# nanoporetech/vbz_compression

Hardware: AMD Instinct MI355X
Metric: MB/s encode+decode, int16 signal, 1/2/4/8 MI355X vs CPU; ratio preserved (higher is better)
Workload: dtype int16

## Files before the change

### vbz_compression_amd/csrc/vbz_api.hip

```cpp
#include <hip/hip_runtime.h>

#include <cmath>
#include <cstdarg>
#include <cstdio>
#include <cstdlib>
#include <cstring>
#include <condition_variable>
#include <mutex>
#include <string>
#include <map>
#include <vector>

#include "../../include/vbz.h"
#include "../../include/vbz_gpu.h"
#include "vbz_kernels.h"

using namespace vbzhip;


struct ProfEntry
{
    const char* name;
    uint32_t launches;
    double ms;
// ... 1905 lines not shown
VBZ_EXPORT int vbz_gpu_x_svb_handover(vbz_gpu_ctx* c, const vbz_gpu_batch* bt, void* plans_out)
{
    if (!c || !bt || !plans_out) return -1;
    DeviceGuard dg(c->device);
    const uint32_t n = bt->n_reads;
    if (n == 0) return 0;
    hipStream_t s = c->stream;
    ReadBatch rb = to_rb(bt);
    uint32_t num, den;
    svb_factor(2, true, &num, &den);
    const size_t scratch_need = (size_t)(((unsigned __int128)bt->src_bytes * num + den - 1) / den) + (size_t)n * 96 + 256;
    StageSlots m;
    if (!ensure(c, c->scratch, scratch_need) || !ensure(c, c->meta, m.carve(nullptr, n)) || !ensure(c, c->encplan, zstd_encode_plan_bytes(n))) return -1;
    m.carve(c->meta.p, n);
    uint64_t* const svb_off = m.svb_off;
    uint32_t *const svb_cap = m.svb_cap, *const svb_size = m.svb_size, *const gate = m.gate;
    HIPCHK(c, launch_plan_scratch(n, bt->src_size, num, den, c->scratch.cap, svb_off, svb_cap, gate, false, s), "plan launch");
    ReadBatch a = rb;
    a.dst = (uint8_t*)c->scratch.p;
    a.dst_off = svb_off;
    a.dst_cap = svb_cap;
    a.result = svb_size;
    a.gate = gate;
    HIPCHK(c, launch_svb_encode(a, 2, true, 0, false, false, nullptr, c->encplan.p, s), "svb_encode launch");
    ReadBatch cp = rb;
    cp.src = (const uint8_t*)c->scratch.p;
    cp.src_off = svb_off;
    cp.src_size = svb_size;
    cp.gate = gate;
    HIPCHK(c, launch_copy_bytes(cp, 0, s), "copy launch");
    HIPCHK(c, hipMemcpyAsync(plans_out, c->encplan.p, (size_t)n * sizeof(EncPlan), hipMemcpyDeviceToDevice, s), "plan copy");
    return 0;
}
#endif

void vbz_gpu_profile_enable(vbz_gpu_ctx* c, int enable)
{
    if (!c) return;
    if (!enable) drain_profile(c);
    c->profiling = enable != 0;
    if (c->half) vbz_gpu_profile_enable(c->half, enable);
}

int vbz_gpu_decode_span_paths(vbz_gpu_ctx* c, uint32_t* by_spans)
{
    if (!c) return -1;
    DeviceGuard guard(c->device);
    if (by_spans) *by_spans = 0;
    if (c->last_span_frames == 0) return 0;
    std::vector<uint32_t> redo(c->last_span_frames);
    if (hipMemcpyAsync(redo.data(), c->last_span_redo, 4ull * redo.size(), hipMemcpyDeviceToHost, c->stream) != hipSuccess) return -1;
    if (hipStreamSynchronize(c->stream) != hipSuccess) return -1;
    uint32_t nb = 0;
    for (uint32_t v : redo) nb += v == 0;
    if (by_spans) *by_spans = nb;
    return (int)c->last_span_frames;
}

static int decode_paths_one(vbz_gpu_ctx* c, uint32_t* batched, uint32_t* walked);

int vbz_gpu_decode_paths(vbz_gpu_ctx* c, uint32_t* batched, uint32_t* walked)
{
    if (!c) return -1;
    uint32_t b0 = 0, w0 = 0, b1 = 0, w1 = 0;
    const int n0 = decode_paths_one(c, &b0, &w0);
    const int n1 = (n0 >= 0 && c->last_split && c->half) ? decode_paths_one(c->half, &b1, &w1) : 0;
// ... 417 lines not shown
```

### vbz_compression_amd/csrc/vbz_kernels.h

```cpp
#pragma once

#include <hip/hip_runtime.h>
#include <stdint.h>

namespace vbzhip {

constexpr uint32_t E_ZSTD = 0xFFFFFFFFu;
constexpr uint32_t E_INPUT_SIZE = 0xFFFFFFFEu;
constexpr uint32_t E_INTEGER_SIZE = 0xFFFFFFFDu;
constexpr uint32_t E_DESTINATION_SIZE = 0xFFFFFFFCu;
constexpr uint32_t E_STREAM = 0xFFFFFFFBu;
constexpr uint32_t E_VERSION = 0xFFFFFFFAu;
constexpr uint32_t E_OOM = 0xFFFFFFF9u;
constexpr uint32_t E_DEVICE = 0xFFFFFFF8u;
constexpr uint32_t E_FIRST = E_DEVICE;
constexpr uint32_t GATE_SKIP = E_FIRST - 1u;
constexpr int PHASE_SLOTS = 12;

constexpr uint32_t SIG_NONE = 0, SIG_F32 = 1, SIG_F16 = 2, SIG_BF16 = 3;
constexpr uint32_t SIG_CHUNK = 4;
constexpr uint32_t SIG_COUNT = 8;
constexpr uint32_t SIG_RANGE = 16;
constexpr uint32_t SIG_TRIM = 32;
constexpr uint32_t RANGE_STATS_RANGE = 0, RANGE_STATS_READ = 1;
// ... 246 lines not shown
    const RefLits* lits = nullptr;
    const uint32_t* lits_pos = nullptr;
    uint32_t lits_units = 0;
};

size_t zstd_ref_pre_bytes(uint32_t n_reads);
const RefPre* zstd_ref_pre(const void* pre_meta);
size_t zstd_ref_table_bytes(uint32_t n_reads);
hipError_t launch_zstd_ref_chain(const ReadBatch& b, const uint32_t* redo, void* pre_meta, void* tables, void* recs, uint64_t recs_cap, RefChains* out,
                                 hipStream_t s);
hipError_t launch_zstd_decode_only(const ReadBatch& b, uint32_t toosmall_code, const void* seq_dtables, const uint32_t* only, RefChains chains,
                                   unsigned long long* dbg, hipStream_t s);
size_t zstd_fast_meta_bytes(uint32_t n_reads);
const RefLits* zstd_ref_lits(const void* lit_meta, uint32_t n_reads);
bool zstd_ref_literals_enabled();
const uint32_t* zstd_fast_redo(const void* meta, uint32_t n_reads);
struct RefWork
{
    void *pre = nullptr, *tables = nullptr, *recs = nullptr;
    uint64_t recs_cap = 0;
    void* lits = nullptr;
    uint32_t lit_units = 0;
};
struct FastDecodeArgs
{
    uint32_t toosmall_code = 0;
    const void* seq_dtables = nullptr;
    void* meta = nullptr;
    RefWork ref;
    unsigned long long* dbg = nullptr;
    FastSide side;
};
hipError_t launch_zstd_decode_fast(const ReadBatch& b, const FastDecodeArgs& a, hipStream_t s);
size_t zstd_ref_lit_meta_bytes(uint32_t n_reads);
uint32_t zstd_ref_lit_units();
const uint32_t* zstd_ref_lit_skip(const void* lit_meta, uint32_t n_reads);
size_t seq_dtables_bytes();
void seq_dtables_build(void* host_buffer);
struct SpanDecodeArgs
{
    uint32_t toosmall_code = 0;
    const void* seq_dtables = nullptr;
    uint64_t content_bytes = 0;
    void* meta = nullptr;
    const uint32_t* redo = nullptr;
};
size_t zstd_dspan_meta_bytes(uint64_t content_bytes, uint32_t n_reads);
hipError_t launch_zstd_decode_spans(const ReadBatch& b, SpanDecodeArgs* a, hipStream_t s);

hipError_t launch_xxh64_batch(const uint8_t* src, const uint64_t* off, const uint32_t* len, const uint32_t* gate, const uint32_t* skip, uint32_t n,
                              uint64_t* out, hipStream_t s);
hipError_t launch_xxh64_verify(const ReadBatch& b, hipStream_t s);
hipError_t launch_checksum_insert(const ReadBatch& b, const uint64_t* hash, uint32_t hdr, const uint32_t* raw_size, uint32_t integer_size, hipStream_t s);

hipError_t launch_pack_layout(uint32_t n, const uint32_t* result, const uint64_t* dst_off, const uint32_t* dst_cap, uint64_t dst_bytes, uint32_t align,
                              uint64_t* packed_off, uint32_t* packed_size, hipStream_t s);
hipError_t launch_sized_layout(uint32_t n, const uint8_t* src, const uint64_t* src_off, const uint32_t* src_size, uint64_t src_bytes, uint32_t align,
                               uint32_t* raw_size, uint64_t* raw_off, hipStream_t s);
hipError_t launch_pack_gather(uint32_t n, const uint8_t* dst, const uint64_t* dst_off, const uint64_t* packed_off, const uint32_t* packed_size,
                              uint8_t* packed, uint64_t packed_cap, hipStream_t s);

hipError_t launch_plan_scratch(uint32_t n, const uint32_t* raw_size, uint32_t mul_num, uint32_t mul_den, uint64_t limit,
                               uint64_t* off, uint32_t* cap, uint32_t* gate, bool gate_is_input, hipStream_t s);
struct ScratchPlan
{
    uint32_t num, den;
// ... 108 lines not shown
```

### vbz_compression_amd/csrc/zstd_decode_fast.hip

```cpp
#include <algorithm>
#include <cstdlib>

#include "vbz_kernels.h"
#include "zstd_runs.h"
#include "zstd_frame.h"
#include "zstd_tables.h"

namespace vbzhip {

namespace {

constexpr uint32_t FAST_TASKS = 64;
constexpr uint32_t TASK_REL = 1u << 31, TASK_TAB = 1u << 30, TASK_CNT = TASK_TAB - 1u;

struct FastFrame
{
    uint32_t fcs, ntask, ntree, block_max;
    uint32_t tree_off[2], tree_len[2];
    uint32_t tlog[2], nw[2];
    uint32_t seq_off, seq_len, nseq;
    uint32_t b0_regen, base_out;
    uint32_t ws_lit, ws_pairs;
    uint32_t cp_off, cp_count, cp_spacing;
    uint32_t blk, lit_csize;
// ... 813 lines not shown
                    if (k0 + 1024u * c + 16u <= mq) v[u][c] = *(gl4*)(f + k0 + 1024u * c);
                const uint32_t rb = mq & 15u;
                tailb[u] = (uint32_t)lane < rb ? f[mq - rb + (uint32_t)lane] : 0u;
            }
#pragma unroll
            for (int u = 0; u < MG; ++u) {
                const uint32_t mq = (uint32_t)__builtin_amdgcn_readlane((int)m, g + u);
                gu8* d = (gu8*)dst + (uint32_t)__builtin_amdgcn_readlane((int)dpos, g + u);
#pragma unroll
                for (int c = 0; c < 3; ++c)
                    if (k0 + 1024u * c + 16u <= mq) *(gst4*)(d + k0 + 1024u * c) = v[u][c];
                const uint32_t rb = mq & 15u;
                if ((uint32_t)lane < rb) d[mq - rb + (uint32_t)lane] = (uint8_t)tailb[u];
                if (mq > 3072u + 16u) {
                    gcu8* f = (gcu8*)(tb + (uint64_t)(g + u) * pcap);
                    for (uint32_t k = k0 + 3072u; k + 16u <= mq; k += 1024u) *(gst4*)(d + k) = *(gl4*)(f + k);
                }
            }
        }
        res.tail = tail_end;
    } else if (F->noseq) {
        LEAVE();
    }
    res.blk = F->blk;
    res.regen = regen;
    res.csize = F->lit_csize;
    res.at = F->ws_lit;
    res.tb = (uint32_t)(tb - (uint64_t)dst);
    res.pcap = pcap;
    LEAVE();
#undef LEAVE
}

constexpr uint32_t RUNS_LDS = 8704;
__global__ __launch_bounds__(WAVE) void fast_runs_kernel(ReadBatch b, const FastFrame* frames, const SeqDTables* dtabs, uint32_t* redo)
{
    __shared__ __attribute__((aligned(16))) uint32_t lds[RUNS_LDS / 4];
    const int lane = threadIdx.x;
    const uint32_t r = blockIdx.x;
    if (redo[r]) return;
    const FastFrame* F = frames + r;
    const uint32_t nseq = F->nseq;
    if (nseq == 0) return;
    const uint8_t* src = b.src + b.src_off[r];
    uint8_t* dst = b.dst + b.dst_off[r];
    const uint2 llt = dtabs->ll[lane], mlt = dtabs->ml[lane];
    uint2* pairs = reinterpret_cast<uint2*>(dst + F->ws_pairs);
    const uint32_t regen = F->b0_regen, base_out = F->base_out;
    uint32_t total = 0, ok = 3;
    if (F->cp_count)
        ok = zero_run_chain_segments(src + F->seq_off, F->seq_len, pairs, nseq, llt, mlt, regen, src + F->cp_off, F->cp_count, F->cp_spacing, lane, &total, lds,
                                     RUNS_LDS);
    if (ok == 3) ok = zero_run_chain(src + F->seq_off, F->seq_len, pairs, nseq, llt, mlt, 6, 6, regen, lane, &total);
    if (ok != 1 || total != base_out) {
        if (lane == 0) redo[r] = 1;
        return;
    }
    __syncthreads();
    const uint32_t end = place_zero_runs(dst, pairs, nseq, dst + F->ws_lit, 2u, regen, 0u, F->fcs, F->block_max, reinterpret_cast<uint8_t*>(lds), RUNS_LDS - 8u, lane);
    if (lane == 0) {
        if (end != base_out) redo[r] = 1;
        else b.result[r] = F->fcs;
    }
}

}

static uint32_t ref_units_max()
{
    static const uint32_t v = [] {
        const char* e = getenv("VBZ_HIP_REF_UNITS");
        const int k = e ? atoi(e) : (int)4;
        return (uint32_t)(k < 1 ? 1 : (k > 4 ? 4 : k));
    }();
    return v;
}

static int ref_lits_ahead()
{
    static const int on = [] {
        const char* e = getenv("VBZ_HIP_REF_LITERALS");
        return e ? atoi(e) : 1;
    }();
    return on;
}

size_t zstd_fast_meta_bytes(uint32_t n_reads)
{
    return (size_t)n_reads * (sizeof(FastFrame) + FAST_TASKS * sizeof(FastTask) + 512 + 4 + 4) + 1024;
}

struct FastMeta
{
    FastFrame* frames;
    FastTask* tasks;
    uint8_t* weights;
    uint32_t* redo;
    uint32_t* scanned;
};
// ... 132 lines not shown
```

### vbz_compression_amd/csrc/zstd_encode.hip

```cpp
#include "vbz_kernels.h"
#include "zstd_entropy.h"
#include "zstd_frame.h"

namespace vbzhip {

namespace {

constexpr int WAVE = 64;
constexpr uint32_t BLOCK_MAX = 128u << 10;
constexpr uint32_t MIN_BLOCK = 4096;
constexpr uint32_t HUF_BLOCK_MAX = 92u << 10;
constexpr uint32_t SPLIT_MIN = 2048;
constexpr int MAXBLK = 16;
#ifndef VBZ_SPAN_BLOCK_KB
#define VBZ_SPAN_BLOCK_KB 16
#endif
constexpr uint32_t SPAN_BLOCK = VBZ_SPAN_BLOCK_KB << 10;
#ifndef VBZ_SPAN_SMALL_BLOCKS
#define VBZ_SPAN_SMALL_BLOCKS 2
#endif
constexpr uint32_t SPAN_BYTES_SMALL = SPAN_BLOCK * VBZ_SPAN_SMALL_BLOCKS, SPAN_BYTES_LARGE = SPAN_BLOCK * MAXBLK;
constexpr uint32_t SPAN_LARGE_FROM = 256u << 20;
#ifndef VBZ_KEYSPAN_KB
#define VBZ_KEYSPAN_KB 8
// ... 1246 lines not shown
    }
}

__device__ __forceinline__ void span_table_role(EncLds& L, SpanRegion* R, int lane)
{
    const uint32_t ns = R->nshared;
    if (ns == 0) return;
    uint32_t mine = 0;
#pragma unroll
    for (int j = 0; j < 4; ++j) {
        const uint32_t c = R->hist[lane + 64 * j];
        L.hist[lane + 64 * j] = c;
        mine += c;
    }
    const uint32_t D = wave_sum_u32(mine);
    wave_lds_sync();
    const uint32_t per = (D + ns - 1) / ns;
    region_plan(L, D, D, ns * ((per + SPAN_BLOCK - 1) / SPAN_BLOCK), lane);
    wave_lds_sync();
#pragma unroll
    for (int j = 0; j < 4; ++j) {
        const uint2 e = L.ctable[lane + 64 * j];
        R->ctable[lane + 64 * j] = e.x | (e.y << 16);
    }
    if (lane < 34) R->tree[lane] = reinterpret_cast<const uint32_t*>(L.tree)[lane];
    if (lane == 0) {
        R->mode = L.mode;
        R->treeSize = (uint32_t)L.treeSize;
        R->huffLog = L.huffLog;
    }
}

#ifndef VBZ_ENC_PACK_WAVES
#define VBZ_ENC_PACK_WAVES 5
#endif
#ifndef VBZ_PACK_PREFETCH
#define VBZ_PACK_PREFETCH 1
#endif
#ifndef VBZ_ENC_WAVES
#define VBZ_ENC_WAVES 4
#endif

template <bool TIMED, bool DEEP, bool TABLES = false>
__global__ __launch_bounds__(WAVE, VBZ_ENC_WAVES) void zstd_encode_kernel(ReadBatch b, const uint32_t* orig_size, uint32_t key_elem,
                                                           const uint32_t* key_bytes, uint32_t hdr, unsigned long long* dbg,
                                                           const uint32_t* src_cap, const SeqCTables* seqtab, const EncSpan* spans,
                                                           const uint32_t* span_count, uint8_t* span_tmp, uint32_t* span_size,
                                                           uint32_t* span_trail, uint32_t trailers, uint32_t* deep_d, EncPlan* plans, uint32_t* redo,
                                                           SpanShared shared)
{
    __shared__ __attribute__((aligned(16))) EncLds L;
    if (TABLES && shared.regions && blockIdx.x >= shared.first_block) {
        span_table_role(L, shared.regions + (blockIdx.x - shared.first_block), threadIdx.x);
        return;
    }
    unsigned long long tph[PHASE_SLOTS] = {};
    unsigned long long tlast = TIMED ? __builtin_readcyclecounter() : 0;
#define PHASE(k) do { if (TIMED) { unsigned long long tn = __builtin_readcyclecounter(); tph[k] += tn - tlast; tlast = tn; } } while (0)
    const int lane = threadIdx.x;
    const bool span_mode = spans != nullptr;
    EncSpan sp = {};
    if (span_mode) {
        if (blockIdx.x >= *span_count) return;
        sp = spans[blockIdx.x];
        if (sp.flags & SPAN_SHARED) return;
        if (lane == 0) { span_size[blockIdx.x] = 0; span_trail[blockIdx.x] = 0; }
        if (sp.flags & SPAN_SKIP) return;
// ... 815 lines not shown
            if (!jsingle) {
                uint8_t* tp = bp + 3 + lh + tsz;
                put_le(tp, s0, 2);
                put_le(tp + 2, s1, 2);
                put_le(tp + 4, s2, 2);
            }
        }
    };
    uint32_t ocur = opos;
    uint32_t spos = 0;
    uint32_t curblk = 0xFFFFFFFFu;
    if (st < 4 * nb) load_chunk(s_beg(st), s_cnt(st), 0, cur);
    PPHASE(1);
    uint32_t base_bits = 0;
    uint32_t flushed = 0;
    uint32_t cb = 0;
    uint32_t pend_fq = 0;
    uint8_t* pend_dst = nullptr;
    auto flush_pending = [&]() {
        uint4* pq = reinterpret_cast<uint4*>(L.obuf[cb ^ 1u]);
        for (uint32_t q = lane; q < pend_fq; q += WAVE) {
            const uint4 v = pq[q];
            pq[q] = make_uint4(0u, 0u, 0u, 0u);
            __builtin_memcpy(pend_dst + 16u * q, &v, 16);
        }
        pend_fq = 0;
    };
    while (st < 4 * nb) {
        if ((st >> 2) != curblk) {
            curblk = st >> 2;
            const uint32_t tsz = curblk == 0 ? treeSize : 0u;
            const uint32_t hl = 3u + blk_lh(curblk) + tsz + (blk_bs(curblk) < 256u ? 0u : 6u);
            if ((uint64_t)ocur + hl > limit) REDO();
            for (uint32_t i = lane; i < tsz; i += WAVE) out[ocur + 3u + blk_lh(curblk) + i] = reinterpret_cast<const uint8_t*>(L.tree)[i];
            spos = ocur + hl;
        }
        const uint32_t scnt = s_cnt(st);
        uint8_t* sop = out + spos;
        uint32_t nst = st, ndone = done + STEP_SYMS;
        if (ndone >= scnt) {
            ndone = 0;
            ++nst;
            while (nst < 4 * nb && s_cnt(nst) == 0) ++nst;
        }
        flush_pending();
#if VBZ_PACK_PREFETCH
        if (nst < 4 * nb) load_chunk(s_beg(nst), s_cnt(nst), ndone, nxt);
#endif
        const int32_t room = (int32_t)(scnt - done) - STEP_LANE * lane;
        const int skip = room >= STEP_LANE ? 0 : (room <= 0 ? STEP_LANE : (int)(STEP_LANE - room));
        uint32_t ent[STEP_LANE];
#pragma unroll
        for (int k = 0; k < STEP_LANE; ++k) ent[k] = mytable[(cur[k >> 2] >> (8 * (k & 3))) & 0xFF];
        if (skip != 0) {
#pragma unroll
            for (int k = 0; k < STEP_LANE; ++k) ent[k] = k >= skip ? ent[k] : 0u;
        }
        uint32_t Tb = 0;
#pragma unroll
        for (int k = 0; k < STEP_LANE; ++k) Tb += ent[k];
        Tb >>= 16;
        const uint32_t incl = wave_incl_scan_u32(Tb);
        const uint32_t total = (uint32_t)__builtin_amdgcn_readlane((int)incl, 63);
        const uint32_t allbits = base_bits + total;
        const uint32_t fq = allbits >> 7;
        if ((uint64_t)spos + flushed + 16ull * fq + 24 > limit) REDO();
        PPHASE(2);
// ... 66 lines not shown
#pragma unroll
        for (int k = 0; k < STEP_DW; ++k) cur[k] = nxt[k];
#else
        if (nst < 4 * nb) load_chunk(s_beg(nst), s_cnt(nst), ndone, cur);
#endif
        st = nst;
        done = ndone;
        PPHASE(5);
    }
    flush_pending();
    if (seqmode && curblk != 0xFFFFFFFFu) {
        wave_lds_sync();
        if ((uint64_t)spos + seqBytes > seqOff) REDO();
        for (uint32_t i = 16u * (uint32_t)lane; i < seqBytes; i += 16u * WAVE) {
            uint4 v;
            __builtin_memcpy(&v, out + seqOff + i, 16);
            if (i + 16u <= seqBytes) __builtin_memcpy(out + spos + i, &v, 16);
            else {
                const uint32_t w[4] = { v.x, v.y, v.z, v.w };
                for (uint32_t k = i; k < seqBytes; ++k) out[spos + k] = (uint8_t)(w[(k - i) >> 2] >> (8 * ((k - i) & 3)));
            }
        }
        wave_lds_sync();
        block_headers(curblk, ocur, seqBytes);
        ocur = spos + seqBytes;
    }
    opos = ocur;
    return true;
#undef PPHASE
#undef REDO
}

template <bool TIMED>
__global__ __launch_bounds__(WAVE, VBZ_ENC_PACK_WAVES) void zstd_pack_kernel(ReadBatch b, const uint32_t* orig_size, uint32_t key_elem, const uint32_t* key_bytes,
                                                                             uint32_t hdr, uint32_t trailers, const EncPlan* plans, uint32_t* redo,
                                                                             unsigned long long* dbg_)
{
    unsigned long long* const dbg = TIMED ? dbg_ : nullptr;
    __shared__ __attribute__((aligned(16))) PackLds L;
    unsigned long long tph[PHASE_SLOTS] = {};
    unsigned long long tlast = TIMED ? __builtin_readcyclecounter() : 0;
#define PPHASE(k) do { if (TIMED) { unsigned long long tn = __builtin_readcyclecounter(); tph[k] += tn - tlast; tlast = tn; } } while (0)
    const int lane = threadIdx.x;
    const uint32_t r = blockIdx.x;
    if (redo[r] != PLAN_READY) return;
#define REDO()                          \
    do {                                \
        if (lane == 0) redo[r] = 0;     \
        return;                         \
    } while (0)
    const uint32_t N = b.src_size[r];
    const uint32_t cap = b.dst_cap[r];
    const uint8_t* in = b.src + b.src_off[r];
    uint8_t* out = b.dst + b.dst_off[r];
    const EncPlan* FP = &plans[r];
    uint32_t K = 0;
    if (N >= SPLIT_MIN) {
        if (key_bytes) K = key_bytes[r];
        else if (key_elem) K = (orig_size[r] / key_elem + 3u) >> 2;
        if (K >= N) K = 0;
    }
    const uint32_t seqBytes = FP->seqBytes, seqOff = FP->seqOff;
    const uint32_t limit = seqBytes ? seqOff : cap;
    uint32_t opos = 0;
    if ((uint64_t)hdr + 9 > limit) REDO();
    if (lane == 0) {
        if (hdr) put_le(out, orig_size[r], 4);
        uint8_t* p = out + hdr;
        put_le(p, ZSTD_MAGIC, 4);
        if (N < 256) { p[4] = 0x20; p[5] = (uint8_t)N; }
        else if (N < 65536 + 256) { p[4] = 0x60; put_le(p + 5, N - 256, 2); }
        else { p[4] = 0xA0; put_le(p + 5, N, 4); }
    }
    opos = hdr + 5 + (N < 256 ? 1 : (N < 65536 + 256 ? 2 : 4));
    PPHASE(0);
    for (int region = 0; region < 2; ++region) {
        if (region == 1 && K == 0) break;
        const uint32_t r0 = region == 0 ? 0u : K;
        const uint32_t r1 = region == 0 ? (K ? K : N) : N;
        const EncRegionPlan* P = &FP->reg[region];
        const uint32_t S = P->S, Sh = P->Sh;
        const uint32_t opos_region = opos;
        if (!pack_region<TIMED>(L, in + r0, r0, out, opos, limit, P->ctable, P->tree, S, P->nblk, P->treeSize, P->seqmode != 0, r1 == N, seqBytes, seqOff, lane,
                                tph, tlast))
            REDO();
        if (Sh != S && opos - opos_region > S + (S >> 6) + 256u) REDO();
        PPHASE(6);
    }
    if (FP->cpCount != 0 && (trailers & 1u)) {
        const uint32_t count = FP->cpCount, tb = 8u + 4u + 4u * count + 4u;
        if ((uint64_t)opos + tb <= cap) {
            __syncthreads();
            uint8_t* tp = out + opos;
            if (lane == 0) {
                put_le(tp, CP_MAGIC, 4);
                put_le(tp + 4, tb - 8u, 4);
                put_le(tp + 8, FP->cpSpacing | (count << 16), 4);
                put_le(tp + 12 + 4 * count, tb, 4);
            }
            if ((uint32_t)lane < count) put_le(tp + 12 + 4 * lane, FP->cp[lane], 4);
            opos += tb;
        }
    }
    if (lane == 0) b.result[r] = opos;
    PPHASE(7);
    if (TIMED && lane == 0)
        for (int k = 0; k < PHASE_SLOTS; ++k) dbg[(size_t)r * PHASE_SLOTS + k] = tph[k];
#undef PPHASE
#undef REDO
}


__global__ __launch_bounds__(1024) void zstd_span_plan_kernel(uint32_t n, const uint32_t* svb_size, const uint32_t* orig_size, uint32_t key_elem,
                                                              const uint32_t* gate, uint32_t seq_enabled, uint32_t max_spans, uint64_t tmp_limit,
                                                              EncSpan* spans, uint32_t* span_first, uint32_t* span_count, SpanRegion* regions, uint32_t shspan)
{
// ... 82 lines not shown
                EncSpan e = {};
                e.read = base + q;
                bool keyseq = false;
                if (j < kN) {
                    e.r0 = (uint32_t)((uint64_t)qK * j / kN);
                    e.r1 = (uint32_t)((uint64_t)qK * (j + 1) / kN);
                    keyseq = keyseq1;
                    e.tmp_off = q_off[q] + (uint64_t)j * slotK;
                    e.tmp_cap = slotK;
                } else {
                    const uint32_t t = j - kN;
                    e.r0 = qK + (uint32_t)((uint64_t)D * t / dN);
                    e.r1 = qK + (uint32_t)((uint64_t)D * (t + 1) / dN);
                    e.tmp_off = q_off[q] + (uint64_t)kN * slotK + (uint64_t)t * slotD;
                    e.tmp_cap = slotD;
                    keyseq = dataseq;
                    if (q_shared[q]) e.flags = SPAN_SHARED | (t == 0 ? SPAN_TREE : 0u);
                }
                e.flags |= (j == 0 ? SPAN_FIRST : 0u) | (j + 1 == cntq ? SPAN_LAST : 0u) | (keyseq ? SPAN_KEYSEQ : 0u);
                e.ord = j;
                spans[si + j] = e;
            }
        }
        __syncthreads();
        if (tid == 1023) { carry_c = pc + ci; carry_b = pb + bi; }
        __syncthreads();
    }
    if (tid == 0) {
        span_first[n] = carry_c;
        *span_count = carry_c < max_spans ? carry_c : max_spans;
    }
}

__global__ __launch_bounds__(WAVE, VBZ_ENC_PACK_WAVES) void zstd_span_pack_kernel(ReadBatch b, const EncSpan* spans, const uint32_t* span_count, uint8_t* span_tmp,
                                                                                  uint32_t* span_size, uint32_t* span_trail, const SpanRegion* regions)
{
    __shared__ __attribute__((aligned(16))) PackLds L;
    const int lane = threadIdx.x;
    if (blockIdx.x >= *span_count) return;
    const EncSpan sp = spans[blockIdx.x];
    if ((sp.flags & (SPAN_SHARED | SPAN_SKIP)) != SPAN_SHARED) return;
    const SpanRegion* R = &regions[sp.read];
    const uint8_t* in = b.src + b.src_off[sp.read];
    uint8_t* out = span_tmp + sp.tmp_off;
    const uint32_t S = sp.r1 - sp.r0, cap = sp.tmp_cap;
    const uint32_t nblk = (S + SPAN_BLOCK - 1) / SPAN_BLOCK;
    const bool last = (sp.flags & SPAN_LAST) != 0, tree = (sp.flags & SPAN_TREE) != 0;
    const uint32_t mode = R->mode;
    uint32_t opos = 0;
    bool packed = false;
    if (mode == 2u) {
        unsigned long long tph[PHASE_SLOTS] = {}, tlast = 0;
        packed = pack_region<false>(L, in + sp.r0, sp.r0, out, opos, cap, R->ctable, R->tree, S, nblk, tree ? R->treeSize : 0u, false, last, 0u, 0u, lane, tph, tlast);
        if (packed && !tree && opos > S + 3u * nblk) packed = false;
        if (!packed && tree) {
            if (lane == 0) { span_size[blockIdx.x] = E_ZSTD; span_trail[blockIdx.x] = 0; }
            return;
        }
    }
    if (!packed) {
        if ((uint64_t)S + 3ull * nblk > cap) {
            if (lane == 0) { span_size[blockIdx.x] = E_ZSTD; span_trail[blockIdx.x] = 0; }
            return;
        }
        wave_lds_sync();
        const uint32_t base = S / nblk, extra = S % nblk;
        const bool rle = mode == 1u;
// ... 366 lines not shown
```

### vbz_compression_amd/csrc/zstd_runs.h

```cpp
#pragma once
#include "vbz_kernels.h"

namespace vbzhip {
namespace {

constexpr int WAVE = 64;
constexpr uint32_t BLOCK_MAX = 128u << 10;

__device__ const int16_t LL_DEFAULT[36] = { 4, 3, 2, 2, 2, 2, 2, 2, 2, 2, 2, 2, 2, 1, 1, 1, 2, 2,
                                            2, 2, 2, 2, 2, 2, 2, 3, 2, 1, 1, 1, 1, 1, -1, -1, -1, -1 };
__device__ const int16_t ML_DEFAULT[53] = { 1, 4, 3, 2, 2, 2, 2, 2, 2, 1, 1, 1, 1, 1, 1, 1, 1, 1, 1, 1, 1, 1, 1, 1, 1, 1, 1,
                                            1, 1, 1, 1, 1, 1, 1, 1, 1, 1, 1, 1, 1, 1, 1, 1, 1, 1, 1, -1, -1, -1, -1, -1, -1, -1 };
__device__ const int16_t OF_DEFAULT[29] = { 1, 1, 1, 1, 1, 1, 2, 2, 2, 1, 1, 1, 1, 1, 1, 1, 1, 1, 1, 1, 1, 1, 1, 1, -1, -1, -1, -1, -1 };
__device__ const uint32_t LL_BASE[36] = { 0, 1, 2, 3, 4, 5, 6, 7, 8, 9, 10, 11, 12, 13, 14, 15, 16, 18,
                                          20, 22, 24, 28, 32, 40, 48, 64, 128, 256, 512, 1024, 2048, 4096, 8192, 16384, 32768, 65536 };
__device__ const uint8_t LL_BITS[36] = { 0, 0, 0, 0, 0, 0, 0, 0, 0, 0, 0, 0, 0, 0, 0, 0, 1, 1,
                                         1, 1, 2, 2, 3, 3, 4, 6, 7, 8, 9, 10, 11, 12, 13, 14, 15, 16 };
__device__ const uint32_t ML_BASE[53] = { 3, 4, 5, 6, 7, 8, 9, 10, 11, 12, 13, 14, 15, 16, 17, 18, 19, 20,
                                          21, 22, 23, 24, 25, 26, 27, 28, 29, 30, 31, 32, 33, 34, 35, 37, 39, 41,
                                          43, 47, 51, 59, 67, 83, 99, 131, 259, 515, 1027, 2051, 4099, 8195, 16387, 32771, 65539 };
__device__ const uint8_t ML_BITS[53] = { 0, 0, 0, 0, 0, 0, 0, 0, 0, 0, 0, 0, 0, 0, 0, 0, 0, 0, 0, 0, 0, 0, 0, 0, 0, 0, 0,
                                         0, 0, 0, 0, 0, 1, 1, 1, 1, 2, 2, 3, 3, 4, 4, 5, 7, 8, 9, 10, 11, 12, 13, 14, 15, 16 };

__device__ __forceinline__ int hbit(uint32_t v) { return 31 - __clz((int)v); }
__device__ __forceinline__ uint32_t uni(uint32_t v) { return (uint32_t)__builtin_amdgcn_readfirstlane((int)v); }
__device__ __forceinline__ uint32_t lane_get(uint32_t v, uint32_t l) { return (uint32_t)__builtin_amdgcn_readlane((int)v, (int)l); }

__device__ __noinline__ uint32_t place_zero_runs(uint8_t* dst, const uint2* pairs, uint32_t nseq, const uint8_t* litp, uint32_t ltype,
                                    uint32_t regen, uint32_t opos, uint32_t fcs, uint32_t block_max, uint8_t* lds_lit,
                                    uint32_t lds_cap, int lane)
{
    const uint8_t rle_byte = ltype == 1 ? litp[0] : 0;
    uint32_t lposw = 0, oposw = opos;
    uint2 pnext = (uint32_t)lane < nseq ? pairs[lane] : make_uint2(0u, 0u);
    for (uint32_t base = 0; base < nseq; base += WAVE) {
        const uint32_t ll = pnext.x, ml = pnext.y;
        {
            const uint32_t i1 = base + WAVE + (uint32_t)lane;
            pnext = i1 < nseq ? pairs[i1] : make_uint2(0u, 0u);
        }
        const uint32_t il = wave_incl_scan_u32(ll), it = wave_incl_scan_u32(ll + ml);
        const uint32_t tl = (uint32_t)__builtin_amdgcn_readlane((int)il, 63), tt = (uint32_t)__builtin_amdgcn_readlane((int)it, 63);
        if ((uint64_t)lposw + tl > regen || (uint64_t)oposw + tt > fcs) return 0xFFFFFFFFu;
        const uint32_t lit_room = (tl + 15u) & ~15u;
        if (ltype != 1 && 5u * lit_room + tt + 16u <= lds_cap) {
            uint32_t* lds_sh = reinterpret_cast<uint32_t*>(lds_lit + lit_room);
            uint8_t* lds_out = lds_lit + 5u * lit_room;
            wave_lds_sync();
            for (uint32_t j = lane; 4 * j < tl; j += WAVE) {
                uint32_t v;
                __builtin_memcpy(&v, litp + lposw + 4 * j, 4);
                reinterpret_cast<uint32_t*>(lds_lit)[j] = v;
            }
            for (uint32_t j = 4u * (uint32_t)lane; j < lit_room; j += 4u * WAVE) *reinterpret_cast<uint4*>(lds_sh + j) = make_uint4(0u, 0u, 0u, 0u);
            for (uint32_t j = 16u * (uint32_t)lane; j < tt; j += 16u * WAVE) *reinterpret_cast<uint4*>(lds_out + j) = make_uint4(0u, 0u, 0u, 0u);
            wave_lds_sync();
            const uint32_t lo = il - ll, oo = it - (ll + ml);
            const uint32_t mprev = wave_prev_lane_u32(ml);
            if (ll != 0 && lane != 0) lds_sh[lo] = mprev;
            wave_lds_sync();
            uint32_t carry = 0;
            for (uint32_t j0 = 0; j0 < tl; j0 += 8u * WAVE) {
                const uint32_t j = j0 + 8u * (uint32_t)lane;
                uint32_t sh[8], run = 0;
                const uint4 a0 = j < lit_room ? *reinterpret_cast<const uint4*>(lds_sh + j) : make_uint4(0u, 0u, 0u, 0u);
                const uint4 a1 = j + 4 < lit_room ? *reinterpret_cast<const uint4*>(lds_sh + j + 4) : make_uint4(0u, 0u, 0u, 0u);
                const uint32_t dl[8] = { a0.x, a0.y, a0.z, a0.w, a1.x, a1.y, a1.z, a1.w };
#pragma unroll
                for (int k = 0; k < 8; ++k) {
                    run += dl[k];
                    sh[k] = run;
                }
                const uint32_t inc = wave_incl_scan_u32(run);
                const uint32_t before = carry + inc - run;
                uint2 lb = make_uint2(0u, 0u);
                if (j < lit_room) lb = *reinterpret_cast<const uint2*>(lds_lit + j);
#pragma unroll
                for (int k = 0; k < 8; ++k)
                    if (j + k < tl) lds_out[j + k + before + sh[k]] = (uint8_t)((k < 4 ? lb.x : lb.y) >> (8 * (k & 3)));
                carry += (uint32_t)__builtin_amdgcn_readlane((int)inc, 63);
            }
            wave_lds_sync();
            if (ll != 0) {
                const uint8_t lastb = lds_lit[il - 1];
                if (lastb != 0)
                    for (uint32_t k = 0; k < ml; ++k) lds_out[oo + ll + k] = lastb;
            }
            wave_lds_sync();
            uint8_t* g = dst + oposw;
            for (uint32_t j = 16u * (uint32_t)lane; j < tt; j += 16u * WAVE) {
                if (j + 16u <= tt) {
                    const uint4 v = *reinterpret_cast<const uint4*>(lds_out + j);
                    __builtin_memcpy(g + j, &v, 16);
                } else {
                    for (uint32_t k = j; k < tt; ++k) g[k] = lds_out[k];
                }
            }
            lposw += tl;
            oposw += tt;
            continue;
// ... 20 lines not shown
                dst[my_out + k] = lastb;
            }
        }
        my_out += ll;
        if (ml < 64) {
            const uint32_t v4 = (uint32_t)lastb * 0x01010101u;
            uint32_t k = 0;
            for (; k + 4 <= ml; k += 4) __builtin_memcpy(dst + my_out + k, &v4, 4);
            for (; k < ml; ++k) dst[my_out + k] = lastb;
        }
        uint64_t big = __ballot(ml >= 64);
        while (big) {
            const int sl_ = __ffsll((long long)big) - 1;
            big &= big - 1;
            const uint32_t bo = (uint32_t)__builtin_amdgcn_readlane((int)my_out, sl_);
            const uint32_t bl = (uint32_t)__builtin_amdgcn_readlane((int)ml, sl_);
            const uint32_t bv = (uint32_t)__builtin_amdgcn_readlane((int)lastb, sl_);
            for (uint32_t k = lane; k < bl; k += WAVE) dst[bo + k] = (uint8_t)bv;
        }
        lposw += tl;
        oposw += tt;
    }
    const uint32_t rest = regen - lposw;
    if ((uint64_t)oposw + rest > fcs) return 0xFFFFFFFFu;
    if (ltype == 1) {
        for (uint32_t k = lane; k < rest; k += WAVE) dst[oposw + k] = rle_byte;
    } else {
        for (uint32_t k = lane; k < rest; k += WAVE) dst[oposw + k] = litp[lposw + k];
    }
    oposw += rest;
    if (oposw - opos > BLOCK_MAX || oposw - opos > block_max) return 0xFFFFFFFFu;
    return oposw;
}

struct SeqDTables
{
    uint2 ll[64], ml[64];
};


__device__ __noinline__ uint32_t zero_run_chain(const uint8_t* bs_, uint32_t bsn_, uint2* ws, uint32_t nseq_, uint2 llt, uint2 mlt,
                                                uint32_t log_ll_, uint32_t log_ml_, uint32_t regen_, int lane, uint32_t* total_out)
{
    const uint32_t bsn = uni(bsn_), nseq = uni(nseq_), log_ll = uni(log_ll_), log_ml = uni(log_ml_), regen = uni(regen_);
    const uint8_t* bs = reinterpret_cast<const uint8_t*>(((uint64_t)uni((uint32_t)((uint64_t)bs_ >> 32)) << 32) |
                                                         uni((uint32_t)(uint64_t)bs_));
    if (bsn == 0) return 0u;
    uint32_t k0 = 0;
    auto load_window = [&]() -> uint32_t {
        const int64_t off = (int64_t)bsn - 4 * (int64_t)(k0 + (uint32_t)lane + 1);
        uint32_t v = 0;
        if (off >= 0) {
            __builtin_memcpy(&v, bs + off, 4);
        } else if (off > -4) {
            for (int k = 0; k < 4 + (int)off; ++k) v |= (uint32_t)bs[k] << (8 * (k - (int)off));
        }
        return v;
    };
    uint32_t win = load_window();
    const uint32_t top = lane_get(win, 0) >> 24;
    if (top == 0) return 0u;
    const uint32_t hb = (uint32_t)hbit(top);
    int64_t bits_left = (int64_t)(bsn - 1) * 8 + hb;
    uint64_t buf = 0;
    uint32_t have = 0, q = 0;
    auto refill = [&]() {
        if (have <= 32) {
            if (q - k0 == 64) {
                k0 += 64;
                win = load_window();
            }
            const uint32_t d = lane_get(win, q - k0);
            ++q;
            buf |= (uint64_t)d << (32 - have);
            have += 32;
// ... 11 lines not shown
    have -= 8 - hb;
    refill();
    uint32_t sl = take(log_ll);
    uint32_t sm = take(log_ml);
    uint64_t sum_ll = 0, sum_all = 0;
    uint32_t pl = 0, pm = 0;
    for (uint32_t si = 0; si < nseq; ++si) {
        const uint32_t elx = lane_get(llt.x, sl), ely = lane_get(llt.y, sl);
        const uint32_t emx = lane_get(mlt.x, sm), emy = lane_get(mlt.y, sm);
        refill();
        const uint32_t mlen = emx + take((emy >> 16) & 0xFF);
        refill();
        const uint32_t llen = elx + take((ely >> 16) & 0xFF);
        if (llen == 0) return 2u;
        const bool mine = (uint32_t)lane == (si & 63);
        pl = mine ? llen : pl;
        pm = mine ? mlen : pm;
        sum_ll += llen;
        sum_all += (uint64_t)llen + mlen;
        if (si + 1 < nseq) {
            refill();
            sl = (ely & 0xFFFF) + take(ely >> 24);
            sm = (emy & 0xFFFF) + take(emy >> 24);
        }
        if ((si & 63) == 63) ws[(si & ~63u) + (uint32_t)lane] = make_uint2(pl, pm);
    }
    if ((uint32_t)lane < (nseq & 63)) ws[(nseq & ~63u) + (uint32_t)lane] = make_uint2(pl, pm);
    if (bits_left != 0) return 0u;
    if (sum_ll > regen) return 0u;
    if (sum_all + (regen - sum_ll) > BLOCK_MAX) return 0u;
    *total_out = (uint32_t)(sum_all + (regen - sum_ll));
    return 1u;
}

__device__ __noinline__ uint32_t zero_run_chain_segments(const uint8_t* bs, uint32_t bsn, uint2* ws, uint32_t nseq, uint2 llt, uint2 mlt,
                                                         uint32_t regen, const uint8_t* cp, uint32_t ncp, uint32_t spacing, int lane,
                                                         uint32_t* total_out, uint32_t* lds, uint32_t lds_bytes)
{
    const uint32_t CAP = lds_bytes - 16u;
    if (bsn == 0 || bsn > CAP || ncp + 1 > (uint32_t)WAVE || spacing == 0) return 3u;
    if ((uint64_t)(ncp + 1) * spacing < nseq || (uint64_t)ncp * spacing >= nseq) return 3u;
    __syncthreads();
    for (uint32_t i = lane; 4 * i < bsn + 8; i += WAVE) {
        uint32_t v = 0;
        if (4 * i + 4 <= bsn) __builtin_memcpy(&v, bs + 4 * i, 4);
        else for (uint32_t k = 0; 4 * i + k < bsn && k < 4; ++k) v |= (uint32_t)bs[4 * i + k] << (8 * k);
        lds[i] = v;
    }
    __syncthreads();
    auto extract = [&](uint32_t pos, uint32_t nb) -> uint32_t {
        const uint32_t d0 = lds[pos >> 5], d1 = lds[(pos >> 5) + 1];
        const uint32_t x = __builtin_amdgcn_alignbit(d1, d0, pos & 31);
        return nb >= 32 ? x : (x & ((1u << nb) - 1u));
    };
    const uint32_t nseg = ncp + 1;
    const bool active = (uint32_t)lane < nseg;
    uint32_t P = 0, sl = 0, sm = 0, bad = 0, impure = 0;
    if (lane == 0) {
        const uint32_t top = lds[(bsn - 1) >> 2] >> (8 * ((bsn - 1) & 3)) & 0xFF;
        if (top == 0) bad = 1;
        else {
            P = (bsn - 1) * 8 + (uint32_t)hbit(top);
            if (P < 12) bad = 1;
            else {
                sl = extract(P - 6, 6);
                sm = extract(P - 12, 6);
                P -= 12;
            }
        }
    } else if (active) {
        uint32_t w;
        __builtin_memcpy(&w, cp + 4 * (lane - 1), 4);
        P = w & 0xFFFFFu;
        sl = (w >> 20) & 63u;
// ... 22 lines not shown
                const uint32_t mlen = emx + (lnb >= 32 ? 0u : (v >> lnb));
                const uint32_t llen = elx + (lnb >= 32 ? v : (v & ((1u << lnb) - 1u)));
                if (llen == 0) impure = 1;
                ws[i] = make_uint2(llen, mlen);
                sum_ll += llen;
                sum_all += llen + mlen;
                if (sum_all > BLOCK_MAX) bad = 1;
                if (more) {
                    const uint32_t sb = snl + snm;
                    const uint32_t v2 = sb ? extract(P - sb, sb) : 0u;
                    P -= sb;
                    sl = (ely & 0xFFFF) + (v2 >> snm);
                    sm = (emy & 0xFFFF) + (v2 & ((1u << snm) - 1u));
                }
            }
        }
    }
    const uint32_t nP = (uint32_t)__shfl_down((int)P0, 1, 64), nsl = (uint32_t)__shfl_down((int)sl0, 1, 64),
                   nsm = (uint32_t)__shfl_down((int)sm0, 1, 64);
    if (active) {
        if ((uint32_t)lane + 1 < nseg) bad |= (P != nP || sl != nsl || sm != nsm) ? 1u : 0u;
        else bad |= P != 0 ? 1u : 0u;
    }
    if (__any(bad)) return 3u;
    if (__any(impure)) return 2u;
    const uint32_t tll = (uint32_t)__builtin_amdgcn_readlane((int)wave_incl_scan_u32(active ? sum_ll : 0u), 63);
    const uint32_t tall = (uint32_t)__builtin_amdgcn_readlane((int)wave_incl_scan_u32(active ? sum_all : 0u), 63);
    if (tll > regen) return 0u;
    if ((uint64_t)tall + (regen - tll) > BLOCK_MAX) return 0u;
    *total_out = tall + (regen - tll);
    __syncthreads();
    return 1u;
}

}
}
```

Before: 624,200.

## Inline runs helpers, shrink runs LDS, tune pack occupancy and 16-bit shift scratch

Turns the zero-run decode helpers into force-inlined variants inside fast_runs_kernel and lowers its LDS from 8704 to 6400 bytes with a six-wave launch bound. place_zero_runs now stores match-length shifts as 16-bit values in LDS, so the literal path needs less scratch space. On the encode side the untimed pack kernel's occupancy hint goes from 5 to 8 waves, the span-pack kernel keeps its own knob, and the tree-copy loop is unrolled to a fixed three iterations. The goal is higher occupancy and less call overhead, at the cost of register pressure and possible fallback when a block no longer fits the smaller LDS. Optional atomic counters behind VBZ_EXPERIMENTS are added for profiling.

```diff
diff --git a/vbz_compression_amd/csrc/vbz_api.hip b/vbz_compression_amd/csrc/vbz_api.hip
--- a/vbz_compression_amd/csrc/vbz_api.hip
+++ b/vbz_compression_amd/csrc/vbz_api.hip
@@ -1961,6 +1961,14 @@
     HIPCHK(c, hipMemcpyAsync(plans_out, c->encplan.p, (size_t)n * sizeof(EncPlan), hipMemcpyDeviceToDevice, s), "plan copy");
     return 0;
 }
+VBZ_EXPORT int vbz_gpu_x_runs_counts(vbz_gpu_ctx* c, unsigned long long* out4, int reset)
+{
+    if (!c || !out4) return -1;
+    DeviceGuard dg(c->device);
+    HIPCHK(c, hipStreamSynchronize(c->stream), "runs counts sync");
+    HIPCHK(c, zstd_fast_runs_counts(out4, reset != 0), "runs counts");
+    return 0;
+}
 #endif
 
 void vbz_gpu_profile_enable(vbz_gpu_ctx* c, int enable)
diff --git a/vbz_compression_amd/csrc/vbz_kernels.h b/vbz_compression_amd/csrc/vbz_kernels.h
--- a/vbz_compression_amd/csrc/vbz_kernels.h
+++ b/vbz_compression_amd/csrc/vbz_kernels.h
@@ -302,6 +302,9 @@
     FastSide side;
 };
 hipError_t launch_zstd_decode_fast(const ReadBatch& b, const FastDecodeArgs& a, hipStream_t s);
+#ifdef VBZ_EXPERIMENTS
+hipError_t zstd_fast_runs_counts(unsigned long long out[4], bool reset);
+#endif
 size_t zstd_ref_lit_meta_bytes(uint32_t n_reads);
 uint32_t zstd_ref_lit_units();
 const uint32_t* zstd_ref_lit_skip(const void* lit_meta, uint32_t n_reads);
diff --git a/vbz_compression_amd/csrc/zstd_decode_fast.hip b/vbz_compression_amd/csrc/zstd_decode_fast.hip
--- a/vbz_compression_amd/csrc/zstd_decode_fast.hip
+++ b/vbz_compression_amd/csrc/zstd_decode_fast.hip
@@ -869,8 +869,20 @@
 #undef LEAVE
 }
 
-constexpr uint32_t RUNS_LDS = 8704;
-__global__ __launch_bounds__(WAVE) void fast_runs_kernel(ReadBatch b, const FastFrame* frames, const SeqDTables* dtabs, uint32_t* redo)
+#ifndef VBZ_RUNS_LDS
+#define VBZ_RUNS_LDS 6400
+#endif
+#ifndef VBZ_RUNS_WAVES
+#define VBZ_RUNS_WAVES 6
+#endif
+constexpr uint32_t RUNS_LDS = VBZ_RUNS_LDS;
+#ifdef VBZ_EXPERIMENTS
+__device__ unsigned long long runs_counts[4];
+#define RUNS_COUNTS runs_counts
+#else
+#define RUNS_COUNTS nullptr
+#endif
+__global__ __launch_bounds__(WAVE, VBZ_RUNS_WAVES) void fast_runs_kernel(ReadBatch b, const FastFrame* frames, const SeqDTables* dtabs, uint32_t* redo)
 {
     __shared__ __attribute__((aligned(16))) uint32_t lds[RUNS_LDS / 4];
     const int lane = threadIdx.x;
@@ -886,15 +898,15 @@
     const uint32_t regen = F->b0_regen, base_out = F->base_out;
     uint32_t total = 0, ok = 3;
     if (F->cp_count)
-        ok = zero_run_chain_segments(src + F->seq_off, F->seq_len, pairs, nseq, llt, mlt, regen, src + F->cp_off, F->cp_count, F->cp_spacing, lane, &total, lds,
-                                     RUNS_LDS);
-    if (ok == 3) ok = zero_run_chain(src + F->seq_off, F->seq_len, pairs, nseq, llt, mlt, 6, 6, regen, lane, &total);
+        ok = zero_run_chain_segments_inl(src + F->seq_off, F->seq_len, pairs, nseq, llt, mlt, regen, src + F->cp_off, F->cp_count, F->cp_spacing, lane, &total, lds,
+                                         RUNS_LDS, RUNS_COUNTS);
+    if (ok == 3) ok = zero_run_chain_inl(src + F->seq_off, F->seq_len, pairs, nseq, llt, mlt, 6, 6, regen, lane, &total);
     if (ok != 1 || total != base_out) {
         if (lane == 0) redo[r] = 1;
         return;
     }
     __syncthreads();
-    const uint32_t end = place_zero_runs(dst, pairs, nseq, dst + F->ws_lit, 2u, regen, 0u, F->fcs, F->block_max, reinterpret_cast<uint8_t*>(lds), RUNS_LDS - 8u, lane);
+    const uint32_t end = place_zero_runs_inl(dst, pairs, nseq, dst + F->ws_lit, 2u, regen, 0u, F->fcs, F->block_max, reinterpret_cast<uint8_t*>(lds), RUNS_LDS - 8u, lane, RUNS_COUNTS);
     if (lane == 0) {
         if (end != base_out) redo[r] = 1;
         else b.result[r] = F->fcs;
@@ -902,6 +914,18 @@
 }
 
 }
+
+#ifdef VBZ_EXPERIMENTS
+hipError_t zstd_fast_runs_counts(unsigned long long out[4], bool reset)
+{
+    hipError_t e = hipMemcpyFromSymbol(out, HIP_SYMBOL(runs_counts), sizeof(runs_counts));
+    if (e == hipSuccess && reset) {
+        const unsigned long long zero[4] = { 0, 0, 0, 0 };
+        e = hipMemcpyToSymbol(HIP_SYMBOL(runs_counts), zero, sizeof(zero));
+    }
+    return e;
+}
+#endif
 
 static uint32_t ref_units_max()
 {
diff --git a/vbz_compression_amd/csrc/zstd_encode.hip b/vbz_compression_amd/csrc/zstd_encode.hip
--- a/vbz_compression_amd/csrc/zstd_encode.hip
+++ b/vbz_compression_amd/csrc/zstd_encode.hip
@@ -1302,7 +1302,13 @@
 }
 
 #ifndef VBZ_ENC_PACK_WAVES
-#define VBZ_ENC_PACK_WAVES 5
+#define VBZ_ENC_PACK_WAVES 8
+#endif
+#ifndef VBZ_ENC_PACK_WAVES_TIMED
+#define VBZ_ENC_PACK_WAVES_TIMED 5
+#endif
+#ifndef VBZ_ENC_SPAN_PACK_WAVES
+#define VBZ_ENC_SPAN_PACK_WAVES 5
 #endif
 #ifndef VBZ_PACK_PREFETCH
 #define VBZ_PACK_PREFETCH 1
@@ -2184,7 +2190,12 @@
             const uint32_t tsz = curblk == 0 ? treeSize : 0u;
             const uint32_t hl = 3u + blk_lh(curblk) + tsz + (blk_bs(curblk) < 256u ? 0u : 6u);
             if ((uint64_t)ocur + hl > limit) REDO();
-            for (uint32_t i = lane; i < tsz; i += WAVE) out[ocur + 3u + blk_lh(curblk) + i] = reinterpret_cast<const uint8_t*>(L.tree)[i];
+            static_assert(sizeof(L.tree) <= 3 * WAVE, "a tree description is three bytes per lane at most");
+#pragma unroll
+            for (uint32_t i0 = 0; i0 < 3 * WAVE; i0 += WAVE) {
+                const uint32_t i = i0 + (uint32_t)lane;
+                if (i < tsz) out[ocur + 3u + blk_lh(curblk) + i] = reinterpret_cast<const uint8_t*>(L.tree)[i];
+            }
             spos = ocur + hl;
         }
         const uint32_t scnt = s_cnt(st);
@@ -2317,7 +2328,7 @@
 }
 
 template <bool TIMED>
-__global__ __launch_bounds__(WAVE, VBZ_ENC_PACK_WAVES) void zstd_pack_kernel(ReadBatch b, const uint32_t* orig_size, uint32_t key_elem, const uint32_t* key_bytes,
+__global__ __launch_bounds__(WAVE, TIMED ? VBZ_ENC_PACK_WAVES_TIMED : VBZ_ENC_PACK_WAVES) void zstd_pack_kernel(ReadBatch b, const uint32_t* orig_size, uint32_t key_elem, const uint32_t* key_bytes,
                                                                              uint32_t hdr, uint32_t trailers, const EncPlan* plans, uint32_t* redo,
                                                                              unsigned long long* dbg_)
 {
@@ -2366,7 +2377,9 @@
         const EncRegionPlan* P = &FP->reg[region];
         const uint32_t S = P->S, Sh = P->Sh;
         const uint32_t opos_region = opos;
-        if (!pack_region<TIMED>(L, in + r0, r0, out, opos, limit, P->ctable, P->tree, S, P->nblk, P->treeSize, P->seqmode != 0, r1 == N, seqBytes, seqOff, lane,
+        int rlane = lane;
+        asm volatile("" : "+v"(rlane));
+        if (!pack_region<TIMED>(L, in + r0, r0, out, opos, limit, P->ctable, P->tree, S, P->nblk, P->treeSize, P->seqmode != 0, r1 == N, seqBytes, seqOff, rlane,
                                 tph, tlast))
             REDO();
         if (Sh != S && opos - opos_region > S + (S >> 6) + 256u) REDO();
@@ -2515,7 +2528,7 @@
     }
 }
 
-__global__ __launch_bounds__(WAVE, VBZ_ENC_PACK_WAVES) void zstd_span_pack_kernel(ReadBatch b, const EncSpan* spans, const uint32_t* span_count, uint8_t* span_tmp,
+__global__ __launch_bounds__(WAVE, VBZ_ENC_SPAN_PACK_WAVES) void zstd_span_pack_kernel(ReadBatch b, const EncSpan* spans, const uint32_t* span_count, uint8_t* span_tmp,
                                                                                   uint32_t* span_size, uint32_t* span_trail, const SpanRegion* regions)
 {
     __shared__ __attribute__((aligned(16))) PackLds L;
diff --git a/vbz_compression_amd/csrc/zstd_runs.h b/vbz_compression_amd/csrc/zstd_runs.h
--- a/vbz_compression_amd/csrc/zstd_runs.h
+++ b/vbz_compression_amd/csrc/zstd_runs.h
@@ -26,9 +26,9 @@
 __device__ __forceinline__ uint32_t uni(uint32_t v) { return (uint32_t)__builtin_amdgcn_readfirstlane((int)v); }
 __device__ __forceinline__ uint32_t lane_get(uint32_t v, uint32_t l) { return (uint32_t)__builtin_amdgcn_readlane((int)v, (int)l); }
 
-__device__ __noinline__ uint32_t place_zero_runs(uint8_t* dst, const uint2* pairs, uint32_t nseq, const uint8_t* litp, uint32_t ltype,
-                                    uint32_t regen, uint32_t opos, uint32_t fcs, uint32_t block_max, uint8_t* lds_lit,
-                                    uint32_t lds_cap, int lane)
+__device__ __forceinline__ uint32_t place_zero_runs_inl(uint8_t* dst, const uint2* pairs, uint32_t nseq, const uint8_t* litp, uint32_t ltype,
+                                                        uint32_t regen, uint32_t opos, uint32_t fcs, uint32_t block_max, uint8_t* lds_lit,
+                                                        uint32_t lds_cap, int lane, unsigned long long* count = nullptr)
 {
     const uint8_t rle_byte = ltype == 1 ? litp[0] : 0;
     uint32_t lposw = 0, oposw = opos;
@@ -43,29 +43,30 @@
         const uint32_t tl = (uint32_t)__builtin_amdgcn_readlane((int)il, 63), tt = (uint32_t)__builtin_amdgcn_readlane((int)it, 63);
         if ((uint64_t)lposw + tl > regen || (uint64_t)oposw + tt > fcs) return 0xFFFFFFFFu;
         const uint32_t lit_room = (tl + 15u) & ~15u;
-        if (ltype != 1 && 5u * lit_room + tt + 16u <= lds_cap) {
-            uint32_t* lds_sh = reinterpret_cast<uint32_t*>(lds_lit + lit_room);
-            uint8_t* lds_out = lds_lit + 5u * lit_room;
+        if (count && lane == 0) atomicAdd(&count[0], 1ull);
+        if (ltype != 1 && 3u * lit_room + tt + 16u <= lds_cap && lds_cap <= 0xFFFFu) {
+            uint16_t* lds_sh = reinterpret_cast<uint16_t*>(lds_lit + lit_room);
+            uint8_t* lds_out = lds_lit + 3u * lit_room;
+            if (count && lane == 0) atomicAdd(&count[1], 1ull);
             wave_lds_sync();
             for (uint32_t j = lane; 4 * j < tl; j += WAVE) {
                 uint32_t v;
                 __builtin_memcpy(&v, litp + lposw + 4 * j, 4);
                 reinterpret_cast<uint32_t*>(lds_lit)[j] = v;
             }
-            for (uint32_t j = 4u * (uint32_t)lane; j < lit_room; j += 4u * WAVE) *reinterpret_cast<uint4*>(lds_sh + j) = make_uint4(0u, 0u, 0u, 0u);
+            for (uint32_t j = 8u * (uint32_t)lane; j < lit_room; j += 8u * WAVE) *reinterpret_cast<uint4*>(lds_sh + j) = make_uint4(0u, 0u, 0u, 0u);
             for (uint32_t j = 16u * (uint32_t)lane; j < tt; j += 16u * WAVE) *reinterpret_cast<uint4*>(lds_out + j) = make_uint4(0u, 0u, 0u, 0u);
             wave_lds_sync();
             const uint32_t lo = il - ll, oo = it - (ll + ml);
             const uint32_t mprev = wave_prev_lane_u32(ml);
-            if (ll != 0 && lane != 0) lds_sh[lo] = mprev;
+            if (ll != 0 && lane != 0) lds_sh[lo] = (uint16_t)mprev;
             wave_lds_sync();
             uint32_t carry = 0;
             for (uint32_t j0 = 0; j0 < tl; j0 += 8u * WAVE) {
                 const uint32_t j = j0 + 8u * (uint32_t)lane;
                 uint32_t sh[8], run = 0;
-                const uint4 a0 = j < lit_room ? *reinterpret_cast<const uint4*>(lds_sh + j) : make_uint4(0u, 0u, 0u, 0u);
-                const uint4 a1 = j + 4 < lit_room ? *reinterpret_cast<const uint4*>(lds_sh + j + 4) : make_uint4(0u, 0u, 0u, 0u);
-                const uint32_t dl[8] = { a0.x, a0.y, a0.z, a0.w, a1.x, a1.y, a1.z, a1.w };
+                const uint4 a = j < lit_room ? *reinterpret_cast<const uint4*>(lds_sh + j) : make_uint4(0u, 0u, 0u, 0u);
+                const uint32_t dl[8] = { a.x & 0xFFFFu, a.x >> 16, a.y & 0xFFFFu, a.y >> 16, a.z & 0xFFFFu, a.z >> 16, a.w & 0xFFFFu, a.w >> 16 };
 #pragma unroll
                 for (int k = 0; k < 8; ++k) {
                     run += dl[k];
@@ -152,6 +153,12 @@
     if (oposw - opos > BLOCK_MAX || oposw - opos > block_max) return 0xFFFFFFFFu;
     return oposw;
 }
+__device__ __noinline__ uint32_t place_zero_runs(uint8_t* dst, const uint2* pairs, uint32_t nseq, const uint8_t* litp, uint32_t ltype,
+                                                 uint32_t regen, uint32_t opos, uint32_t fcs, uint32_t block_max, uint8_t* lds_lit,
+                                                 uint32_t lds_cap, int lane)
+{
+    return place_zero_runs_inl(dst, pairs, nseq, litp, ltype, regen, opos, fcs, block_max, lds_lit, lds_cap, lane);
+}
 
 struct SeqDTables
 {
@@ -159,8 +166,8 @@
 };
 
 
-__device__ __noinline__ uint32_t zero_run_chain(const uint8_t* bs_, uint32_t bsn_, uint2* ws, uint32_t nseq_, uint2 llt, uint2 mlt,
-                                                uint32_t log_ll_, uint32_t log_ml_, uint32_t regen_, int lane, uint32_t* total_out)
+__device__ __forceinline__ uint32_t zero_run_chain_inl(const uint8_t* bs_, uint32_t bsn_, uint2* ws, uint32_t nseq_, uint2 llt, uint2 mlt,
+                                                       uint32_t log_ll_, uint32_t log_ml_, uint32_t regen_, int lane, uint32_t* total_out)
 {
     const uint32_t bsn = uni(bsn_), nseq = uni(nseq_), log_ll = uni(log_ll_), log_ml = uni(log_ml_), regen = uni(regen_);
     const uint8_t* bs = reinterpret_cast<const uint8_t*>(((uint64_t)uni((uint32_t)((uint64_t)bs_ >> 32)) << 32) |
@@ -238,14 +245,22 @@
     *total_out = (uint32_t)(sum_all + (regen - sum_ll));
     return 1u;
 }
-
-__device__ __noinline__ uint32_t zero_run_chain_segments(const uint8_t* bs, uint32_t bsn, uint2* ws, uint32_t nseq, uint2 llt, uint2 mlt,
-                                                         uint32_t regen, const uint8_t* cp, uint32_t ncp, uint32_t spacing, int lane,
-                                                         uint32_t* total_out, uint32_t* lds, uint32_t lds_bytes)
+__device__ __noinline__ uint32_t zero_run_chain(const uint8_t* bs, uint32_t bsn, uint2* ws, uint32_t nseq, uint2 llt, uint2 mlt,
+                                                uint32_t log_ll, uint32_t log_ml, uint32_t regen, int lane, uint32_t* total_out)
+{
+    return zero_run_chain_inl(bs, bsn, ws, nseq, llt, mlt, log_ll, log_ml, regen, lane, total_out);
+}
+
+__device__ __forceinline__ uint32_t zero_run_chain_segments_inl(const uint8_t* bs, uint32_t bsn, uint2* ws, uint32_t nseq, uint2 llt, uint2 mlt,
+                                                                uint32_t regen, const uint8_t* cp, uint32_t ncp, uint32_t spacing, int lane,
+                                                                uint32_t* total_out, uint32_t* lds, uint32_t lds_bytes,
+                                                                unsigned long long* count = nullptr)
 {
     const uint32_t CAP = lds_bytes - 16u;
+    if (count && lane == 0) atomicAdd(&count[2], 1ull);
     if (bsn == 0 || bsn > CAP || ncp + 1 > (uint32_t)WAVE || spacing == 0) return 3u;
     if ((uint64_t)(ncp + 1) * spacing < nseq || (uint64_t)ncp * spacing >= nseq) return 3u;
+    if (count && lane == 0) atomicAdd(&count[3], 1ull);
     __syncthreads();
     for (uint32_t i = lane; 4 * i < bsn + 8; i += WAVE) {
         uint32_t v = 0;
@@ -334,6 +349,12 @@
     __syncthreads();
     return 1u;
 }
-
-}
-}
+__device__ __noinline__ uint32_t zero_run_chain_segments(const uint8_t* bs, uint32_t bsn, uint2* ws, uint32_t nseq, uint2 llt, uint2 mlt,
+                                                         uint32_t regen, const uint8_t* cp, uint32_t ncp, uint32_t spacing, int lane,
+                                                         uint32_t* total_out, uint32_t* lds, uint32_t lds_bytes)
+{
+    return zero_run_chain_segments_inl(bs, bsn, ws, nseq, llt, mlt, regen, cp, ncp, spacing, lane, total_out, lds, lds_bytes);
+}
+
+}
+}
```

Result: faster. 641,700, median of 6 (+2.8%).
